# MAGIC-SCAN/adipose_tissue-unet

Hardware: AMD Instinct MI355X
Metric: 1024^2 tiles/sec (train) (higher is better)
Workload: dtype bf16; 1 GPU; unet_bn L5 base64 1024x1024x3 bf16 B=4/GPU (BASELINE configs[2]); preset=unet_bn, levels=5, tile=1024, batch_per_gpu=4, global_batch=4, parallelism=dp1

## Files before the change

### adipose_tissue-unet_amd/csrc/conv_fwd_halo.hip

```cpp
#include <type_traits>

#include "conv_common.h"

namespace {

__device__ __attribute__((aligned(256))) uint4 halo_zero_page[64];

constexpr int PH = 8, PW = 32;
constexpr int HH = PH + 2, HW = PW + 2;
constexpr int HROWS = HH * HW;
constexpr int ROWB = 128;

__device__ __forceinline__ int hswz(int r) { return r & 7; }

#define LDS_BAR()                                             \
  do {                                                        \
    asm volatile("s_waitcnt lgkmcnt(0)" ::: "memory");        \
    __builtin_amdgcn_s_barrier();                             \
    asm volatile("" ::: "memory");                            \
  } while (0)

#define HALO_BAR()                         \
  do {                                     \
    asm volatile("" ::: "memory");         \
    __builtin_amdgcn_s_barrier();          \
    asm volatile("" ::: "memory");         \
  } while (0)

template <int WN, int KS, int TPS, int NHB>
constexpr int halo_lds() {
  constexpr int NTH = 4 * WN * KS * 64;
  constexpr int GH = (HROWS * 8 + NTH - 1) / NTH;
  return NHB * (GH * NTH / 8) * ROWB + 3 * TPS * WN * 64 * ROWB;
}

template <int WN, int KS, int TPS, int NHB, bool BNR>
__global__ __launch_bounds__(4 * WN * KS * 64, (halo_lds<WN, KS, TPS, NHB>() <= 81920 ? 2 : 1))
void igemm_fwd_halo_kernel(FwdArgs a) {
  constexpr int NTH = 4 * WN * KS * 64;
  constexpr int BN = WN * 64;
  constexpr int SPC = (9 + TPS - 1) / TPS;
  constexpr int GH = (HROWS * 8 + NTH - 1) / NTH;
  constexpr int HROWS_PAD = GH * NTH / 8;
  constexpr int HBUF = HROWS_PAD * ROWB;
  constexpr int GB1 = BN * 8 / NTH;
  static_assert(GB1 * NTH == BN * 8, "weight slot must split evenly");
  constexpr int GB = GB1 * TPS;
  constexpr int WTAP = BN * ROWB;
  constexpr int WSLOT = TPS * WTAP;
  constexpr int OFF_W = NHB * HBUF;
  constexpr int LT = BN + 4;
  constexpr int EPI = PH * PW * LT * 4;
  constexpr int SMEM = (OFF_W + 3 * WSLOT > EPI) ? OFF_W + 3 * WSLOT : EPI;
  __shared__ __attribute__((aligned(1024))) unsigned char smem[SMEM];

  const int tid = threadIdx.x, lane = tid & 63;
  const int wave = __builtin_amdgcn_readfirstlane(tid >> 6);
  const int wm = wave % 4, wn = (wave / 4) % WN, kh = wave / (4 * WN);
  const int tx_n = a.Wo / PW, ty_n = a.Ho / PH;
  const int lin = xcd_remap(blockIdx.x, a.nblocks);
  const int tn = lin % a.ntile_n;
  int rest = lin / a.ntile_n;
  const int px = rest % tx_n; rest /= tx_n;
  const int py = rest % ty_n;
  const int img = rest / ty_n;
  const int y0 = py * PH, x0 = px * PW, n0 = tn * BN;
  const int Cin_s = a.CAs + a.CBs;
  const int nchunk = Cin_s / 64, nsteps = nchunk * SPC;
  const int Wrows = (a.Nout + 63) / 64 * 64;
  const bf16* srcA = reinterpret_cast<const bf16*>(a.srcA);
  const bf16* srcB = reinterpret_cast<const bf16*>(a.srcB);

  int hoff[GH], hcol[GH];
#pragma unroll
  for (int i = 0; i < GH; ++i) {
    const int idx = i * NTH + tid;
    const int hr = idx >> 3, pos = idx & 7;
    hcol[i] = 8 * (pos ^ hswz(hr));
    const int gy = y0 - 1 + hr / HW, gx = x0 - 1 + hr % HW;
    hoff[i] = (hr < HROWS && gy >= 0 && gy < a.Hs && gx >= 0 && gx < a.Ws) ? (img * a.Hs + gy) * a.Ws + gx : -1;
  }
  const bf16* wp[GB1];
#pragma unroll
  for (int i = 0; i < GB1; ++i) {
    const int idx = i * NTH + tid;
    const int q = idx >> 3, pos = idx & 7;
    wp[i] = (n0 + q < Wrows) ? reinterpret_cast<const bf16*>(a.W) + (size_t)(n0 + q) * a.Kpad + 8 * (pos ^ swz(q))
                             : nullptr;
  }

  auto issue_halo = [&](int c, int buf) {
    const int ci = c * 64;
    const bf16* base = ci < a.CAs ? srcA + ci : srcB + (ci - a.CAs);
    const int cs = ci < a.CAs ? a.CAs : a.CBs;
    unsigned char* dst = smem + buf * HBUF + wave * 8 * ROWB;
#pragma unroll
    for (int i = 0; i < GH; ++i) {
      const void* p = hoff[i] >= 0 ? (const void*)(base + (size_t)hoff[i] * cs + hcol[i]) : (const void*)halo_zero_page;
      __builtin_amdgcn_global_load_lds(p, (lds_void*)(dst + i * (NTH / 8) * ROWB), 16, 0, 0);
    }
  };
  auto issue_w = [&](int s) {
    const int c = s / SPC, j = s - SPC * c;
#pragma unroll
    for (int u = 0; u < TPS; ++u) {
      const int t = j * TPS + u;
      const int k = t * Cin_s + c * 64;
      unsigned char* dst = smem + OFF_W + (s % 3) * WSLOT + u * WTAP + wave * 8 * ROWB;
#pragma unroll
      for (int i = 0; i < GB1; ++i) {
        const void* p = (wp[i] && t < 9) ? (const void*)(wp[i] + k) : (const void*)halo_zero_page;
        __builtin_amdgcn_global_load_lds(p, (lds_void*)(dst + i * (NTH / 8) * ROWB), 16, 0, 0);
      }
    }
  };

  f32x4 acc[4][4];
#pragma unroll
  for (int i = 0; i < 4; ++i)
#pragma unroll
    for (int j = 0; j < 4; ++j) acc[i][j] = f32x4{0.f, 0.f, 0.f, 0.f};

  const int r16 = lane & 15, h4 = lane >> 4;
  issue_halo(0, 0);
  issue_w(0);
  if (nsteps > 1) {
    issue_w(1);
    asm volatile("s_waitcnt vmcnt(%0)" ::"n"(GB) : "memory");
  } else {
    asm volatile("s_waitcnt vmcnt(0)" ::: "memory");
  }
  HALO_BAR();

  for (int s = 0; s < nsteps; ++s) {
    const int c = s / SPC, j = s - SPC * c;
    const bool nh = NHB == 2 && j == 0 && c + 1 < nchunk;
    if (nh) issue_halo(c + 1, (c + 1) & 1);
    const bool nw = s + 2 < nsteps;
    if (nw) issue_w(s + 2);
    const unsigned char* H = smem + (NHB == 2 ? (c & 1) : 0) * HBUF;
#pragma unroll
    for (int u = 0; u < TPS; ++u) {
    const int t = j * TPS + u;
    if (t >= 9) break;
    const int dy = t / 3, dx = t - 3 * dy;
    const unsigned char* Wt = smem + OFF_W + (s % 3) * WSLOT + u * WTAP;
#pragma unroll
    for (int kq = 0; kq < 2 / KS; ++kq) {
      const int ck = 4 * (KS == 2 ? kh : kq) + h4;
      bf16x8 fb[4], fa[4];
#pragma unroll
      for (int nf = 0; nf < 4; ++nf) {
        const int q = wn * 64 + nf * 16 + r16;
        fb[nf] = *reinterpret_cast<const bf16x8*>(Wt + q * ROWB + ((ck ^ swz(q)) << 4));
      }
#pragma unroll
      for (int mf = 0; mf < 4; ++mf) {
        const int prow = 2 * wm + (mf >> 1), pcol = (mf & 1) * 16 + r16;
        const int hr = (prow + dy) * HW + pcol + dx;
        fa[mf] = *reinterpret_cast<const bf16x8*>(H + hr * ROWB + ((ck ^ hswz(hr)) << 4));
      }
#pragma unroll
      for (int mf = 0; mf < 4; ++mf)
#pragma unroll
        for (int nf = 0; nf < 4; ++nf)
          acc[mf][nf] = __builtin_amdgcn_mfma_f32_16x16x32_bf16(fa[mf], fb[nf], acc[mf][nf], 0, 0, 0);
    }
    }
    if (nw) {
      if (nh) asm volatile("s_waitcnt vmcnt(%0)" ::"n"(GB + GH) : "memory");
      else asm volatile("s_waitcnt vmcnt(%0)" ::"n"(GB) : "memory");
    } else {
      asm volatile("s_waitcnt vmcnt(0)" ::: "memory");
    }
    HALO_BAR();
  }

  float* tile = reinterpret_cast<float*>(smem);
  const int col = lane & 15, rq = (lane >> 4) * 4;
#pragma unroll
  for (int part = 0; part < KS; ++part) {
    if (kh == part) {
#pragma unroll
      for (int mf = 0; mf < 4; ++mf)
#pragma unroll
        for (int nf = 0; nf < 4; ++nf)
#pragma unroll
          for (int r = 0; r < 4; ++r) {
            const int p = (2 * wm + (mf >> 1)) * PW + (mf & 1) * 16 + rq + r;
            float* e = tile + p * LT + wn * 64 + nf * 16 + col;
            *e = part == 0 ? acc[mf][nf][r] : *e + acc[mf][nf][r];
          }
    }
    ADP_LDS_BARRIER();
  }
  float bs[8], bq[8];
#pragma unroll
  for (int j = 0; j < 8; ++j) { bs[j] = 0.f; bq[j] = 0.f; }
  for (int pr = 0; pr < PH; ++pr) {
    const int m0 = (img * a.Ho + y0 + pr) * a.Wo + x0;
    if constexpr (BNR) epi_rows_bnr<NTH, BN>(a, tile + pr * PW * LT, PW, m0, n0, tid, bs, bq);
    else epi_rows<NTH, BN>(a, tile + pr * PW * LT, PW, m0, n0, tid, bs, bq);
  }
  if (a.bn_sum || a.bnr_z) epi_bn_flush<NTH, BN>(a, tile, n0, tid, bs, bq);
}

#ifndef HALOP_VALU_PER_MFMA
#define HALOP_VALU_PER_MFMA 8
#endif
template <int I, int N, typename F>
__device__ __forceinline__ void halop_static_for(F&& f) {
  if constexpr (I < N) {
    f(std::integral_constant<int, I>{});
    halop_static_for<I + 1, N>(f);
  }
}
template <bool BNR, int NCH, int BN, bool PIPE, int EPI_, bool WIDE = false, bool DYN = false, bool SWP = false>
__global__ __launch_bounds__(512, 1) void igemm_fwd_halop_kernel(FwdArgs a) {
  constexpr bool BNL = EPI_ == 6;
  constexpr int EPI = BNL ? 1 : EPI_;
  static_assert(!BNL || (!BNR && !DYN && !SWP && NCH == 1), "BN-on-load: one-chunk static-list forward launches");
  static_assert(!BNR || EPI == 0, "the BN-backward reduction launch stores the plain product");
  static_assert(EPI < 4 || !PIPE, "mask / addend quads, the dropout hash and two accumulator sets: registers");
  constexpr int NTH = 512, NF = BN / 16;
  constexpr int HCH = NCH * HROWS * 8;
  constexpr int GH = (HCH + NTH - 1) / NTH;
  static_assert(!BNL || GH <= 6, "BN-on-load: at most six halo chunks per thread");
  constexpr int HBUF = HCH * 16;
  constexpr int GW = 9 * NCH * BN * 8 / NTH;
  constexpr int WTAP = NCH * BN * ROWB;
  constexpr int OFF_W = HBUF, OFF_C = OFF_W + 9 * WTAP;
  constexpr int OFF_S = OFF_C + 5 * BN * 4 + 16;
  constexpr int SMEM = OFF_S + (BNL ? 2 * NCH * 64 * 4 : 0);
  static_assert(GW * NTH == 9 * NCH * BN * 8, "weights must split evenly");
  static_assert(SMEM <= 160 * 1024, "LDS");
  typedef __bf16 bf16x4 __attribute__((ext_vector_type(4)));
  typedef unsigned int v2u32_h __attribute__((ext_vector_type(2)));
  typedef unsigned int v4u32_h __attribute__((ext_vector_type(4)));
  __shared__ __attribute__((aligned(1024))) unsigned char smem[SMEM];

  const int tid = threadIdx.x, lane = tid & 63;
  const int wave = __builtin_amdgcn_readfirstlane(tid >> 6);
  prio_static<ADP_PRIO_FWD>(wave);
  const int tx_n = a.Wo / PW, ty_n = a.Ho / PH;
  const int T = a.nblocks, G = gridDim.x;
  const int lin = xcd_remap(blockIdx.x, G);
  constexpr bool dyn = DYN;
  const bool full = dyn && a.claim_full;
  const int nt = dyn ? 0 : (lin < T ? (T - lin + G - 1) / G : 0);
  if (!dyn && nt == 0) return;
  const int Wrows = (a.Nout + 63) / 64 * 64;
  const int NT = a.ntile_n;
  const int nh = lin % NT, n0 = BN * nh;
  const bool second = a.out_mode == 2 && n0 >= a.split_c;
  bf16* obase = reinterpret_cast<bf16*>(second ? a.out2 : a.out);
  const int ostride = second ? a.out2_stride : a.out_stride;
  const int ocol0 = second ? n0 - a.split_c : n0;
  const int nlim = a.out_mode == 2 && !second ? a.split_c : a.Nout;
  const int Cin_s = a.CAs + a.CBs;

  int* ring = reinterpret_cast<int*>(smem + OFF_C + 5 * BN * 4);
  const int npatch = T / NT;
  const int CH = dyn ? a.claim_chunk : 1, nsup = (npatch + CH - 1) / CH;
  auto sup_id = [&](int sidx) -> int {
    const int v = full ? claim_ring_read(ring + (sidx & 3))
                       : sidx < 2 ? lin / NT + sidx * (G / NT) : 2 * (G / NT) + claim_ring_read(ring + (sidx & 3));
    return v < nsup ? v : -1;
  };
  auto tile_id = [&](int k) -> int {
    if (!dyn) return k < nt ? lin / NT + k * (G / NT) : -1;
    const int v = sup_id(k / CH);
    const int t = v * CH + k % CH;
    return v >= 0 && t < npatch ? t : -1;
  };
  if (full) {
    if (tid == 0) {
      const int r = claim_next2(a.claim + nh);
      ring[0] = r;
      ring[1] = r + 1;
    }
    __syncthreads();
  }
  if (dyn && tile_id(0) < 0) {
    if (tid == 0) claim_block_done(a.claim, NT, G);
    return;
  }
  auto tile_origin = [&](int t, int& img, int& y0, int& x0) {
    const int px = t % tx_n, r = t / tx_n;
    y0 = (r % ty_n) * PH;
    img = r / ty_n;
    x0 = px * PW;
  };
  auto halo_src = [&](int img, int y0, int x0, int i) -> const uint4* {
    const int idx = i * NTH + tid;
    const int cc = NCH == 1 ? 0 : (idx >= HROWS * 8 ? 1 : 0), hr = (idx - cc * HROWS * 8) >> 3;
    const int hy = hr / HW, hx = hr - hy * HW;
    const int gy = y0 + hy - 1, gx = x0 + hx - 1, us = a.up >> 1;
    const bool ok = (i < GH - 1 || idx < HCH) && (unsigned)gy < (unsigned)(a.Hs << us) && (unsigned)gx < (unsigned)(a.Ws << us);
    if (!ok) return nullptr;
    const bool inA = cc * 64 < a.CAs;
    const bf16* src = reinterpret_cast<const bf16*>(inA ? a.srcA : a.srcB);
    const int cs = inA ? a.CAs : a.CBs;
    return reinterpret_cast<const uint4*>(src + (size_t)((img * a.Hs + (gy >> us)) * a.Ws + (gx >> us)) * cs +
                                          (inA ? cc * 64 : cc * 64 - a.CAs) + 8 * ((tid & 7) ^ hswz(hr)));
  };

  const float* sS = reinterpret_cast<const float*>(smem + OFF_S);
  const bool act_w = BNL && n0 == 0 && a.act_out != nullptr && !(ADP_DBG(a) & 4096);
  const __amdgpu_buffer_rsrc_t rsA = __builtin_amdgcn_make_buffer_rsrc(
      a.act_out, 0, act_w ? a.Nimg * a.Hs * a.Ws * a.CAs * 2 : 0, 0x00020000);
  auto bnl = [&](uint4 v, int img, int y0, int x0, int i) -> uint4 {
    const int idx = i * NTH + tid;
    const int cc = NCH == 1 ? 0 : (idx >= HROWS * 8 ? 1 : 0), hr = (idx - cc * HROWS * 8) >> 3;
    const int hy = hr / HW, hx = hr - hy * HW;
    const int gy = y0 + hy - 1, gx = x0 + hx - 1;
    const bool inimg = (unsigned)gy < (unsigned)a.Hs && (unsigned)gx < (unsigned)a.Ws;
    const int c0 = cc * 64 + 8 * ((tid & 7) ^ hswz(hr));
    Grp<bf16> g;
    g.v = v;
    bf16* e = reinterpret_cast<bf16*>(&g.v);
#pragma unroll
    for (int hv = 0; hv < 2; ++hv) {
      const float4 q = *reinterpret_cast<const float4*>(sS + c0 + 4 * hv);
      const float4 r = *reinterpret_cast<const float4*>(sS + NCH * 64 + c0 + 4 * hv);
      e[4 * hv + 0] = (bf16)fmaxf(fmaf((float)e[4 * hv + 0], q.x, r.x), 0.f);
      e[4 * hv + 1] = (bf16)fmaxf(fmaf((float)e[4 * hv + 1], q.y, r.y), 0.f);
      e[4 * hv + 2] = (bf16)fmaxf(fmaf((float)e[4 * hv + 2], q.z, r.z), 0.f);
      e[4 * hv + 3] = (bf16)fmaxf(fmaf((float)e[4 * hv + 3], q.w, r.w), 0.f);
    }
    const bool wr = inimg && hy >= 1 && hy <= PH && hx >= 1 && hx <= PW;
    const unsigned off = wr ? (unsigned)((((img * a.Hs + gy) * a.Ws + gx) * a.CAs + c0) * 2) : 0x80000000u;
    if (act_w) __builtin_amdgcn_raw_buffer_store_b128(__builtin_bit_cast(v4u32_h, g.v), rsA, off, 0, 0);
    return inimg ? g.v : v;
  };

#pragma unroll
  for (int i = 0; i < GW; ++i) {
    const int idx = i * NTH + tid;
    const int tc = idx / (BN * 8), rem = idx - tc * BN * 8;
    const int t = tc / NCH, cc = tc - t * NCH;
    const int q = rem >> 3, pos = rem & 7;
    const void* p = n0 + q < Wrows
                        ? (const void*)(reinterpret_cast<const bf16*>(a.W) + (size_t)(n0 + q) * a.Kpad + t * Cin_s + cc * 64 +
                                        8 * (pos ^ swz(q)))
                        : (const void*)halo_zero_page;
    __builtin_amdgcn_global_load_lds(p, (lds_void*)(smem + OFF_W + (size_t)(i * NTH + wave * 64) * 16), 16, 0, 0);
  }
  int img0, y00, x00;
  tile_origin(tile_id(0), img0, y00, x00);
#pragma unroll
  for (int i = 0; i < GH; ++i) {
    if (i * NTH + tid < HCH) {
      const uint4* p = halo_src(img0, y00, x00, i);
      __builtin_amdgcn_global_load_lds(p ? (const void*)p : (const void*)halo_zero_page,
                                       (lds_void*)(smem + (size_t)(i * NTH + wave * 64) * 16), 16, 0, 0);
    }
  }
  float* cst = reinterpret_cast<float*>(smem + OFF_C);
  if (tid < BN) {
    const int c = n0 + tid;
    const bool v = c < a.Nout;
    cst[tid] = (!BNR && a.bias && v) ? a.bias[c] : 0.f;
    cst[BN + tid] = (BNR && v) ? a.bnr_sc[c] : 0.f;
    cst[2 * BN + tid] = (BNR && v) ? a.bnr_sh[c] : 0.f;
    cst[3 * BN + tid] = (BNR && v) ? -a.bnr_mean[c] * a.bnr_invstd[c] : 0.f;
    cst[4 * BN + tid] = (BNR && v) ? a.bnr_invstd[c] : 0.f;
  }
  if constexpr (BNL) {
    float* sw = reinterpret_cast<float*>(smem + OFF_S);
    if (tid < NCH * 64) {
      sw[tid] = a.scA[tid];
      sw[NCH * 64 + tid] = a.shA[tid];
    }
  }
  asm volatile("s_waitcnt vmcnt(0)" ::: "memory");
  __syncthreads();
  if constexpr (BNL) {
#pragma unroll
    for (int i = 0; i < GH; ++i)
      if (i * NTH + tid < HCH) {
        uint4* q = reinterpret_cast<uint4*>(smem + (size_t)(i * NTH + tid) * 16);
        *q = bnl(*q, img0, y00, x00, i);
      }
    __syncthreads();
  }

  const int r16 = lane & 15, h4 = lane >> 4;
  constexpr bool stats = BNR || EPI == 1 || EPI == 3;
  float s1[NF][4], s2[NF][4];
#pragma unroll
  for (int nf = 0; nf < NF; ++nf)
#pragma unroll
    for (int i = 0; i < 4; ++i) { s1[nf][i] = 0.f; s2[nf][i] = 0.f; }

  const __amdgpu_buffer_rsrc_t rsO =
      __builtin_amdgcn_make_buffer_rsrc((void*)obase, 0, a.M * ostride * 2, 0x00020000);
  const __amdgpu_buffer_rsrc_t rsZ = __builtin_amdgcn_make_buffer_rsrc(
      (void*)(BNR ? a.bnr_z : a.out), 0, BNR ? a.M * a.bnr_zs * 2 : 0, 0x00020000);
  const void* mptr = second ? a.mask2 : a.mask;
  const int mstr = second ? a.mask2_stride : a.mask_stride;
  const float mscale = second ? a.mask2_scale : a.mask_scale;
  const bool has_mask = EPI == 4 && mptr != nullptr, has_add = EPI == 4 && !second && a.addend != nullptr;
  const __amdgpu_buffer_rsrc_t rsM =
      __builtin_amdgcn_make_buffer_rsrc((void*)mptr, 0, has_mask ? a.M * mstr * 2 : 0, 0x00020000);
  const __amdgpu_buffer_rsrc_t rsD =
      __builtin_amdgcn_make_buffer_rsrc((void*)a.addend, 0, has_add ? a.M * a.addend_stride * 2 : 0, 0x00020000);
  auto load_q = [&](__amdgpu_buffer_rsrc_t rs, int str, int col0, int mrow_, uint2 (&zr)[2][NF]) {
#pragma unroll
    for (int mf = 0; mf < 2; ++mf)
#pragma unroll
      for (int nf = 0; nf < NF; ++nf) {
        const int c0 = nf * 16 + 4 * h4;
        const unsigned off = n0 + c0 < nlim ? (unsigned)(((mrow_ + mf * 16 + r16) * str + col0 + c0) * 2) : 0x80000000u;
        zr[mf][nf] = __builtin_bit_cast(uint2, __builtin_amdgcn_raw_buffer_load_b64(rs, off, 0, 0));
      }
  };
  auto load_z = [&](int mrow_, uint2 (&zr)[2][NF]) {
    if (ADP_DBG(a) & 8192) {
#pragma unroll
      for (int mf = 0; mf < 2; ++mf)
#pragma unroll
        for (int nf = 0; nf < NF; ++nf) zr[mf][nf] = uint2{0u, 0u};
      return;
    }
    load_q(rsZ, a.bnr_zs, n0, mrow_, zr);
  };
  auto epi_vals = [&](int mf, int nf, const f32x4& av, uint2 zv, int mrow_, uint2 dv = uint2{0u, 0u}) -> bf16x4 {
    const int c0 = nf * 16 + 4 * h4;
    const float4 cb = *reinterpret_cast<const float4*>(cst + c0);
    const int m = mrow_ + mf * 16 + r16;
    float v[4] = {av[0] + cb.x, av[1] + cb.y, av[2] + cb.z, av[3] + cb.w};
    if constexpr (EPI == 4) {
      const bf16x4 dd = __builtin_bit_cast(bf16x4, dv), mm = __builtin_bit_cast(bf16x4, zv);
#pragma unroll
      for (int i = 0; i < 4; ++i) {
        if (has_add) v[i] += (float)dd[i];
        if (has_mask) v[i] = (float)mm[i] > 0.f ? v[i] * mscale : 0.f;
      }
    }
    if constexpr (EPI == 5) {
      const float ks = 1.f / (1.f - a.drop_rate);
#pragma unroll
      for (int i = 0; i < 4; ++i) {
        const float u = adp_uniform(a.drop_seed, (uint64_t)m * (uint64_t)a.Nout + (n0 + c0 + i));
        v[i] = u >= a.drop_rate ? fmaxf(v[i], 0.f) * ks : 0.f;
      }
    }
    bf16x4 o;
#pragma unroll
    for (int i = 0; i < 4; ++i) {
      if constexpr (EPI == 2 || EPI == 3) v[i] = fmaxf(v[i], 0.f);
      o[i] = (bf16)v[i];
    }
    if constexpr (BNR) {
      if (ADP_DBG(a) & 16384) return o;
      const float4 sc = *reinterpret_cast<const float4*>(cst + BN + c0);
      const float4 sh = *reinterpret_cast<const float4*>(cst + 2 * BN + c0);
      const float4 nm = *reinterpret_cast<const float4*>(cst + 3 * BN + c0);
      const float4 is = *reinterpret_cast<const float4*>(cst + 4 * BN + c0);
      const float scv[4] = {sc.x, sc.y, sc.z, sc.w}, shv[4] = {sh.x, sh.y, sh.z, sh.w};
      const float nmv[4] = {nm.x, nm.y, nm.z, nm.w}, isv[4] = {is.x, is.y, is.z, is.w};
      bf16x4 zz = __builtin_bit_cast(bf16x4, zv);
#pragma unroll
      for (int i = 0; i < 4; ++i) {
        const float g = (float)o[i], zf = (float)zz[i];
        const float db = fmaf(zf, scv[i], shv[i]) > 0.f ? g : 0.f;
        s1[nf][i] += db;
        s2[nf][i] = fmaf(db, fmaf(zf, isv[i], nmv[i]), s2[nf][i]);
      }
    } else if constexpr (EPI == 1 || EPI == 3) {
#pragma unroll
      for (int i = 0; i < 4; ++i) {
        s1[nf][i] += v[i];
        s2[nf][i] = fmaf(v[i], v[i], s2[nf][i]);
      }
    }
    return o;
  };
  auto epi_unit = [&](int mf, int nf, const f32x4& av, uint2 zv, int mrow_, uint2 dv = uint2{0u, 0u}) {
    const bf16x4 o = epi_vals(mf, nf, av, zv, mrow_, dv);
    const int c0 = nf * 16 + 4 * h4, m = mrow_ + mf * 16 + r16;
    const unsigned off = n0 + c0 < nlim ? (unsigned)((m * ostride + ocol0 + c0) * 2) : 0x80000000u;
    __builtin_amdgcn_raw_buffer_store_b64(__builtin_bit_cast(v2u32_h, o), rsO, off, 0, 0);
  };
  auto epi_join = [&](int mf, int nf, v2u32_h o0, v2u32_h o1, int mrow_) {
    const auto e0 = __builtin_amdgcn_permlane16_swap(o0.x, o1.x, false, false);
    const auto e1 = __builtin_amdgcn_permlane16_swap(o0.y, o1.y, false, false);
    const v4u32_h st = {e0[0], e1[0], e0[1], e1[1]};
    const int cw = 16 * (nf + (h4 & 1)) + 8 * (h4 >> 1), m = mrow_ + mf * 16 + r16;
    const unsigned off = n0 + cw < nlim ? (unsigned)((m * ostride + ocol0 + cw) * 2) : 0x80000000u;
    __builtin_amdgcn_raw_buffer_store_b128(st, rsO, off, 0, 0);
  };
  auto epi_pair = [&](int mf, int nf, const f32x4& av0, const f32x4& av1, uint2 zv0, uint2 zv1, int mrow_,
                      uint2 dv0 = uint2{0u, 0u}, uint2 dv1 = uint2{0u, 0u}) {
    const v2u32_h o0 = __builtin_bit_cast(v2u32_h, epi_vals(mf, nf, av0, zv0, mrow_, dv0));
    const v2u32_h o1 = __builtin_bit_cast(v2u32_h, epi_vals(mf, nf + 1, av1, zv1, mrow_, dv1));
    epi_join(mf, nf, o0, o1, mrow_);
  };
  v2u32_h pend = {0u, 0u};
  auto epi_all = [&](const f32x4 (&av)[2][NF], const uint2 (&zv)[2][NF], int mrow_, const uint2 (&dv)[EPI == 4 ? 2 : 1][NF]) {
    if constexpr (WIDE) {
#pragma unroll
      for (int nf = 0; nf < NF; nf += 2)
#pragma unroll
        for (int mf = 0; mf < 2; ++mf)
          epi_pair(mf, nf, av[mf][nf], av[mf][nf + 1], zv[mf][nf], zv[mf][nf + 1], mrow_, dv[EPI == 4 ? mf : 0][nf],
                   dv[EPI == 4 ? mf : 0][nf + 1]);
    } else {
#pragma unroll
      for (int nf = 0; nf < NF; ++nf)
#pragma unroll
        for (int mf = 0; mf < 2; ++mf) epi_unit(mf, nf, av[mf][nf], zv[mf][nf], mrow_, dv[EPI == 4 ? mf : 0][nf]);
    }
  };

  f32x4 acc[2][NF], accp[2][NF];
  uint2 zreg[2][NF], dreg[EPI == 4 ? 2 : 1][NF];
  int mrowp = 0;
  auto load_halo = [&](int t, uint4 (&hr)[GH]) {
    int img1, y01, x01;
    tile_origin(t, img1, y01, x01);
    const bool nohalo = (ADP_DBG(a) & 1024) != 0;
#pragma unroll
    for (int i = 0; i < GH; ++i) {
      const uint4* p = nohalo ? nullptr : halo_src(img1, y01, x01, i);
      hr[i] = p ? *p : make_uint4(0, 0, 0, 0);
    }
  };
  auto run_tile = [&](int k, int tk, auto with_prev, uint4 (&hreg)[GH]) -> int {
    constexpr bool EPI_PREV = decltype(with_prev)::value;
    if constexpr (!DYN) tk = tile_id(k);
    const int tn = tile_id(k + 1);
    const bool more = tn >= 0;
    const bool claim_now = dyn && k % CH == 0 && more && sup_id(k / CH + 1) >= 0;
    int claimed = 0;
    if (claim_now && tid == 0) claimed = __hip_atomic_fetch_add(a.claim + nh, 1, __ATOMIC_RELAXED, __HIP_MEMORY_SCOPE_AGENT);
    int img, y0, x0;
    tile_origin(tk, img, y0, x0);
    const int mrow = (img * a.Ho + y0 + wave) * a.Wo + x0;
    if constexpr (BNR) load_z(EPI_PREV ? mrowp : mrow, zreg);
    if constexpr (EPI == 4) {
      if (has_mask) load_q(rsM, mstr, ocol0, mrow, zreg);
      if (has_add) load_q(rsD, a.addend_stride, ocol0, mrow, dreg);
    }
    if (more) load_halo(DYN ? tn : tile_id(k + 1), hreg);
    int img1 = 0, y01 = 0, x01 = 0;
    if constexpr (BNL) {
      if (more) tile_origin(tn, img1, y01, x01);
    }
#pragma unroll
    for (int i = 0; i < 2; ++i)
#pragma unroll
      for (int j = 0; j < NF; ++j) acc[i][j] = f32x4{0.f, 0.f, 0.f, 0.f};
    if constexpr (SWP) {
      constexpr int NS = 18 * NCH;
      bf16x8 FB[2][NF], FA[2][2];
      auto ldf = [&](auto sc, bf16x8 (&fb)[NF], bf16x8 (&fa)[2]) {
        constexpr int st = decltype(sc)::value, t = st / (2 * NCH), cc = (st >> 1) % NCH, kq = st & 1;
        constexpr int dy = t / 3, dx = t - 3 * dy;
        const unsigned char* Wt = smem + OFF_W + t * WTAP + cc * BN * ROWB;
        const unsigned char* Hc = smem + cc * HROWS * ROWB;
        const int ck = 4 * kq + h4;
#pragma unroll
        for (int nf = 0; nf < NF; ++nf) {
          const int q = nf * 16 + r16;
          fb[nf] = *reinterpret_cast<const bf16x8*>(Wt + q * ROWB + ((ck ^ swz(q)) << 4));
        }
#pragma unroll
        for (int mf = 0; mf < 2; ++mf) {
          const int hr = (wave + dy) * HW + mf * 16 + r16 + dx;
          fa[mf] = *reinterpret_cast<const bf16x8*>(Hc + hr * ROWB + ((ck ^ hswz(hr)) << 4));
        }
      };
      ldf(std::integral_constant<int, 0>{}, FB[0], FA[0]);
      halop_static_for<0, NS>([&](auto sc) {
        constexpr int st = decltype(sc)::value, t = st / (2 * NCH), cc = (st >> 1) % NCH, kq = st & 1;
        if constexpr (st + 1 < NS) ldf(std::integral_constant<int, st + 1>{}, FB[(st + 1) & 1], FA[(st + 1) & 1]);
        __builtin_amdgcn_sched_barrier(0);
        const bf16x8(&fb)[NF] = FB[st & 1];
        const bf16x8(&fa)[2] = FA[st & 1];
        constexpr bool with_unit = EPI_PREV && cc == 0 && kq == 0 && t >= 1 && t - 1 < 2 * NF;
        if constexpr (with_unit) {
          constexpr int u = t - 1;
          if constexpr (WIDE) {
            constexpr int p = u >> 1, mf = p & 1, nf = 2 * (p >> 1);
            if constexpr ((u & 1) == 0) {
              pend = __builtin_bit_cast(v2u32_h, epi_vals(mf, nf, accp[mf][nf], zreg[mf][nf], mrowp));
            } else {
              epi_join(mf, nf, pend, __builtin_bit_cast(v2u32_h, epi_vals(mf, nf + 1, accp[mf][nf + 1],
                                                                          zreg[mf][nf + 1], mrowp)), mrowp);
            }
          } else {
            epi_unit(u & 1, u >> 1, accp[u & 1][u >> 1], zreg[u & 1][u >> 1], mrowp);
          }
        }
        if constexpr (!with_unit) prio_hi<ADP_PRIO_FWD>();
#pragma unroll
        for (int mf = 0; mf < 2; ++mf)
#pragma unroll
          for (int nf = 0; nf < NF; ++nf)
            acc[mf][nf] = __builtin_amdgcn_mfma_f32_16x16x32_bf16(fb[nf], fa[mf], acc[mf][nf], 0, 0, 0);
        if constexpr (!with_unit) prio_lo<ADP_PRIO_FWD>();
        if constexpr (with_unit) {
#pragma unroll
          for (int i = 0; i < 2 * NF; ++i) {
            __builtin_amdgcn_sched_group_barrier(0x008, 1, 0);
            __builtin_amdgcn_sched_group_barrier(0x002, HALOP_VALU_PER_MFMA, 0);
          }
        }
      });
    }
#pragma unroll
    for (int t = 0; t < (SWP ? 0 : 9); ++t) {
      const int dy = t / 3, dx = t - 3 * dy;
#pragma unroll
      for (int cc = 0; cc < NCH; ++cc) {
        const unsigned char* Wt = smem + OFF_W + t * WTAP + cc * BN * ROWB;
        const unsigned char* Hc = smem + cc * HROWS * ROWB;
#pragma unroll
        for (int kq = 0; kq < 2; ++kq) {
          const int ck = 4 * kq + h4;
          bf16x8 fb[NF], fa[2];
#pragma unroll
          for (int nf = 0; nf < NF; ++nf) {
            const int q = nf * 16 + r16;
            fb[nf] = *reinterpret_cast<const bf16x8*>(Wt + q * ROWB + ((ck ^ swz(q)) << 4));
          }
#pragma unroll
          for (int mf = 0; mf < 2; ++mf) {
            const int hr = (wave + dy) * HW + mf * 16 + r16 + dx;
            fa[mf] = *reinterpret_cast<const bf16x8*>(Hc + hr * ROWB + ((ck ^ hswz(hr)) << 4));
          }
          constexpr bool unit_here = EPI_PREV;
          const bool with_unit = unit_here && cc == 0 && kq == 0 && t >= 1 && t - 1 < 2 * NF;
          if (with_unit) {
            const int u = t - 1;
            if constexpr (WIDE) {
              const int p = u >> 1, mf = p & 1, nf = 2 * (p >> 1);
              if ((u & 1) == 0) {
                pend = __builtin_bit_cast(v2u32_h, epi_vals(mf, nf, accp[mf][nf], zreg[mf][nf], mrowp));
              } else {
                epi_join(mf, nf, pend, __builtin_bit_cast(v2u32_h, epi_vals(mf, nf + 1, accp[mf][nf + 1],
                                                                            zreg[mf][nf + 1], mrowp)), mrowp);
              }
            } else {
              const int mf = u & 1, nf = u >> 1;
              epi_unit(mf, nf, accp[mf][nf], zreg[mf][nf], mrowp);
            }
          }
          const bool with_apply = BNL && kq == 1 && t >= 3 && t - 3 < GH;
          if constexpr (BNL) {
            if (with_apply && more) hreg[t - 3] = bnl(hreg[t - 3], img1, y01, x01, t - 3);
          }
          if (!with_unit && !with_apply) prio_hi<ADP_PRIO_FWD>();
#pragma unroll
          for (int mf = 0; mf < 2; ++mf)
#pragma unroll
            for (int nf = 0; nf < NF; ++nf)
              acc[mf][nf] = __builtin_amdgcn_mfma_f32_16x16x32_bf16(fb[nf], fa[mf], acc[mf][nf], 0, 0, 0);
          if (!with_unit && !with_apply) prio_lo<ADP_PRIO_FWD>();
          if (with_unit || with_apply) {
#pragma unroll
            for (int i = 0; i < 2 * NF; ++i) {
              __builtin_amdgcn_sched_group_barrier(0x008, 1, 0);
              __builtin_amdgcn_sched_group_barrier(0x002, HALOP_VALU_PER_MFMA, 0);
            }
          }
        }
      }
    }
    if constexpr (PIPE) {
#pragma unroll
      for (int i = 0; i < 2; ++i)
#pragma unroll
        for (int j = 0; j < NF; ++j) accp[i][j] = acc[i][j];
      mrowp = mrow;
    } else {
      epi_all(acc, zreg, mrow, dreg);
    }
    if (more) {
      LDS_BAR();
#pragma unroll
      for (int i = 0; i < GH; ++i)
        if (i * NTH + tid < HCH) *reinterpret_cast<uint4*>(smem + (size_t)(i * NTH + tid) * 16) = hreg[i];
      if (claim_now && tid == 0) ring[(k / CH + 2) & 3] = claimed;
      LDS_BAR();
    }
    return DYN ? tn : tile_id(k + 1);
  };
  uint4 hA[GH];
  int tnext = run_tile(0, tile_id(0), std::false_type{}, hA);
  for (int k = 1; tnext >= 0; ++k) tnext = run_tile(k, tnext, std::integral_constant<bool, PIPE>{}, hA);
  if constexpr (PIPE) {
    if constexpr (BNR) load_z(mrowp, zreg);
    epi_all(accp, zreg, mrowp, dreg);
  }
  if (dyn && tid == 0) claim_block_done(a.claim, NT, G);
  if (!stats || (ADP_DBG(a) & 2)) return;
  double* d0 = a.stat + (size_t)((blockIdx.x * 8 + wave) & (adp::STAT_REPL - 1)) * 2 * adp::STAT_CMAX;
#pragma unroll
  for (int nf = 0; nf < NF; ++nf)
#pragma unroll
    for (int i = 0; i < 4; ++i) {
      const float x = row16_sum(s1[nf][i]), y = row16_sum(s2[nf][i]);
      const int c = n0 + nf * 16 + 4 * h4 + i;
      if (r16 == 0 && c < a.Nout) {
        atomicAdd(d0 + c, (double)x);
        atomicAdd(d0 + adp::STAT_CMAX + c, (double)y);
      }
    }
}

#undef HALO_BAR
#undef LDS_BAR

template <int WN, int KS, int TPS, int NHB>
void launch_halo(FwdArgs& a, hipStream_t s) {
  constexpr int BN = WN * 64;
  a.ntile_n = (a.Nout + BN - 1) / BN;
  a.nblocks = a.Nimg * (a.Ho / PH) * (a.Wo / PW) * a.ntile_n;
  adp::set_kernel("igemm_fwd_halo_kernel<%d, %d, %d, %d, %s>", WN, KS, TPS, NHB, a.bnr_z ? "true" : "false");
  const dim3 g(a.nblocks), b(4 * WN * KS * 64);
  if (a.bnr_z) hipLaunchKernelGGL((igemm_fwd_halo_kernel<WN, KS, TPS, NHB, true>), g, b, 0, s, a);
  else hipLaunchKernelGGL((igemm_fwd_halo_kernel<WN, KS, TPS, NHB, false>), g, b, 0, s, a);
}

}

namespace adp {
int launch_fwd_halo(FwdArgs& a, hipStream_t s) {
  const int mode = option("fwd_halo", 1);
  if (mode == 0) return 0;
  const int Cin_s = a.CAs + a.CBs;
  const bool bnl = a.scA != nullptr;
  if (bnl && !(a.act_out && a.CBs == 0 && a.up == 1 && a.CAs == 64 && a.bn_sum && !a.bnr_z &&
               !a.relu && !a.bias && option("halop_bnl", 1)))
    return 0;
  if (a.scB || a.kh != 3 || a.kw != 3 || a.dil != 1 || a.pad != 1 || a.stride != 1 || (a.up != 1 && a.up != 2) ||
      a.Ho != a.Hs * a.up || a.Wo != a.Ws * a.up || a.Ho % PH != 0 || a.Wo % PW != 0 || a.CAs % 64 != 0 || a.CBs % 64 != 0 ||
      a.K != 9 * Cin_s || a.Kpad != a.K || a.Nout > 128)
    return 0;
  if (a.bnr_z && (a.out_mode != 0 || a.bias || a.relu || a.drop_rate > 0.f || a.accum || a.bn_sum)) return 0;
  const bool one_chunk = Cin_s == 64;
  const bool plain = !a.addend && !a.mask && !a.mask2 && !a.accum && a.drop_rate == 0.f && a.out_stride % 8 == 0;
  const bool dropepi = a.drop_rate > 0.f && a.relu && !a.addend && !a.mask && !a.mask2 && !a.accum && !a.bn_sum &&
                       !a.bnr_z && a.out_mode == 0 && a.out_stride % 8 == 0 && option("halop_dropout", 1);
  const bool maskepi = (a.addend || a.mask || a.mask2) && !a.accum && a.drop_rate == 0.f && !a.bnr_z && !a.bn_sum && !a.relu && !a.bias &&
                       a.out_stride % 8 == 0 && (!a.mask || a.mask_stride % 4 == 0) &&
                       (!a.mask2 || a.mask2_stride % 4 == 0) && (!a.addend || a.addend_stride % 4 == 0) &&
                       (size_t)a.M * std::max(std::max(a.mask ? a.mask_stride : 0, a.mask2 ? a.mask2_stride : 0),
                                              a.addend ? a.addend_stride : 0) * 2 < ((size_t)1 << 31) &&
                       option("halop_mask", 1);
  int bn = 0;
  if (one_chunk && (a.Nout <= 64 || a.Nout == 128)) bn = 64;
  else if (Cin_s == 128 && (a.Nout == 64 || a.Nout == 128) && option("halo_persist2", 1)) bn = 32;
  const int nt_n = bn ? (a.Nout + bn - 1) / bn : 1;
  const bool split_ok = a.out_mode == 2 && bn && a.split_c > 0 && a.split_c % bn == 0 && a.split_c < a.Nout &&
                        (!a.mask2 || maskepi) && a.out2_stride % 8 == 0 && (a.Nout - a.split_c) % bn == 0;
  const size_t lim = (size_t)1 << 31;
  const bool fits = (size_t)a.M * a.out_stride * 2 < lim && (!a.out2 || (size_t)a.M * a.out2_stride * 2 < lim) &&
                    (!a.bnr_z || (size_t)a.M * a.bnr_zs * 2 < lim);
  if (bn && (plain || maskepi || dropepi) && fits && (a.out_mode == 0 || split_ok) && option("halo_persist", 1) &&
      (a.up == 1 || !a.bnr_z)) {
    const int tiles = a.Nimg * (a.Ho / PH) * (a.Wo / PW) * nt_n;
    a.ntile_n = nt_n;
    a.nblocks = tiles;
    int grid = std::max(1, std::min(tiles, option("halo_persist_grid", 256)));
    grid -= grid % nt_n;
    if (grid == 0) grid = nt_n;
    const bool bnr = a.bnr_z != nullptr;
    const int pm = option("halop_pipe", 1);
    const int swm = option("halop_swp", 2);
    const bool swp_req = !bnr && !dropepi && (swm == 1 || (swm == 2 && !one_chunk));
    const bool pipe = !swp_req && !bnr && !maskepi && !dropepi && (pm == 2 || (pm == 1 && one_chunk));
    const int epi = bnr ? 0 : dropepi ? 5 : maskepi ? 4 : (a.bn_sum ? 1 : 0) + (a.relu ? 2 : 0);
    const int wm = option("halop_wide", 3);
    const bool wide = !bnr && (wm == 2 || (wm == 1 && !pipe) || (wm == 3 && !(pipe && (epi == 1 || epi == 3)))) &&
                      a.Nout % 8 == 0 && (a.out_mode != 2 || a.split_c % 8 == 0);
    a.claim = option("halop_claim", option("dp_claim", 0)) && nt_n + 1 <= CLAIM_INTS && !(bnr && one_chunk) && !(pipe && (epi == 1 || epi == 3))
                  ? claim_slot() : nullptr;
    a.claim_chunk = std::max(1, option("halop_claim_chunk", 4));
    a.claim_full = 0;
    if (a.claim) {
      const int nsup = (tiles / nt_n + a.claim_chunk - 1) / a.claim_chunk;
      grid = std::max(nt_n, std::min(grid, nsup * nt_n));
      a.claim_full = option("claim_full", 0) && nsup >= 4 * (grid / nt_n);
    }
    if (bnl) a.claim = nullptr;
    const bool dyn = a.claim != nullptr;
    const bool swp = !dyn && swp_req;
    if (bnl) {
      if (one_chunk && a.Nout <= 64 && pipe && !wide && !swp && epi == 1) {
        adp::set_kernel("igemm_fwd_halop_kernel<false, 1, 64, true, 6, false, false, false>");
        hipLaunchKernelGGL((igemm_fwd_halop_kernel<false, 1, 64, true, 6, false, false, false>), dim3(grid), dim3(512), 0,
                           s, a);
        return 1;
      }
      return 0;
    }
    adp::set_kernel("igemm_fwd_halop_kernel<%s, %d, %d, %s, %d, %s, %s, %s>", bnr ? "true" : "false", one_chunk ? 1 : 2, bn,
                    pipe ? "true" : "false", epi, wide ? "true" : "false", dyn ? "true" : "false", swp ? "true" : "false");
#define HALOP_LAUNCH_WD(NCH_, BN_, W_, D_, P_)                                                                   \
  do {                                                                                                      \
    if (bnr) hipLaunchKernelGGL((igemm_fwd_halop_kernel<true, NCH_, BN_, false, 0, false, D_, P_>), dim3(grid), dim3(512), 0, s, a); \
    else if (epi == 4) hipLaunchKernelGGL((igemm_fwd_halop_kernel<false, NCH_, BN_, false, 4, W_, D_, P_>), dim3(grid), dim3(512), 0, s, a); \
    else if (epi == 5) hipLaunchKernelGGL((igemm_fwd_halop_kernel<false, NCH_, BN_, false, 5, W_, D_, P_>), dim3(grid), dim3(512), 0, s, a); \
    else if (pipe) {                                                                                        \
      if (epi == 1) hipLaunchKernelGGL((igemm_fwd_halop_kernel<false, NCH_, BN_, true, 1, W_, D_, P_>), dim3(grid), dim3(512), 0, s, a); \
      else if (epi == 2) hipLaunchKernelGGL((igemm_fwd_halop_kernel<false, NCH_, BN_, true, 2, W_, D_, P_>), dim3(grid), dim3(512), 0, s, a); \
      else if (epi == 3) hipLaunchKernelGGL((igemm_fwd_halop_kernel<false, NCH_, BN_, true, 3, W_, D_, P_>), dim3(grid), dim3(512), 0, s, a); \
      else hipLaunchKernelGGL((igemm_fwd_halop_kernel<false, NCH_, BN_, true, 0, W_, D_, P_>), dim3(grid), dim3(512), 0, s, a); \
    } else {                                                                                                \
      if (epi == 1) hipLaunchKernelGGL((igemm_fwd_halop_kernel<false, NCH_, BN_, false, 1, W_, D_, P_>), dim3(grid), dim3(512), 0, s, a); \
      else if (epi == 2) hipLaunchKernelGGL((igemm_fwd_halop_kernel<false, NCH_, BN_, false, 2, W_, D_, P_>), dim3(grid), dim3(512), 0, s, a); \
      else if (epi == 3) hipLaunchKernelGGL((igemm_fwd_halop_kernel<false, NCH_, BN_, false, 3, W_, D_, P_>), dim3(grid), dim3(512), 0, s, a); \
      else hipLaunchKernelGGL((igemm_fwd_halop_kernel<false, NCH_, BN_, false, 0, W_, D_, P_>), dim3(grid), dim3(512), 0, s, a); \
    }                                                                                                       \
  } while (0)
#define HALOP_LAUNCH_SWP(NCH_, BN_, W_)                                                                         \
  do {                                                                                                      \
    if (epi == 4) hipLaunchKernelGGL((igemm_fwd_halop_kernel<false, NCH_, BN_, false, 4, W_, false, true>), dim3(grid), dim3(512), 0, s, a); \
    else if (epi == 1) hipLaunchKernelGGL((igemm_fwd_halop_kernel<false, NCH_, BN_, false, 1, W_, false, true>), dim3(grid), dim3(512), 0, s, a); \
    else if (epi == 2) hipLaunchKernelGGL((igemm_fwd_halop_kernel<false, NCH_, BN_, false, 2, W_, false, true>), dim3(grid), dim3(512), 0, s, a); \
    else if (epi == 3) hipLaunchKernelGGL((igemm_fwd_halop_kernel<false, NCH_, BN_, false, 3, W_, false, true>), dim3(grid), dim3(512), 0, s, a); \
    else hipLaunchKernelGGL((igemm_fwd_halop_kernel<false, NCH_, BN_, false, 0, W_, false, true>), dim3(grid), dim3(512), 0, s, a); \
  } while (0)
#define HALOP_LAUNCH_W(NCH_, BN_, W_)                          \
  do {                                                         \
    if (dyn) HALOP_LAUNCH_WD(NCH_, BN_, W_, true, false);      \
    else if (swp) HALOP_LAUNCH_SWP(NCH_, BN_, W_);              \
    else HALOP_LAUNCH_WD(NCH_, BN_, W_, false, false);         \
  } while (0)
#define HALOP_LAUNCH(NCH_, BN_)                  \
  do {                                           \
    if (wide) HALOP_LAUNCH_W(NCH_, BN_, true);   \
    else HALOP_LAUNCH_W(NCH_, BN_, false);       \
  } while (0)
    if (one_chunk) HALOP_LAUNCH(1, 64);
    else HALOP_LAUNCH(2, 32);
#undef HALOP_LAUNCH_W
#undef HALOP_LAUNCH_WD
#undef HALOP_LAUNCH_SWP
#undef HALOP_LAUNCH
    return 1;
  }
  if (bnl) return 0;
  if (a.Nout == 128 && Cin_s > 128 && !a.bnr_z && plain && a.out_mode != 1 && option("halo_defer_tap64p", 1))
    return 0;
  if (a.up != 1) return 0;
  if (a.Nout <= 64) {
    if (one_chunk && mode != 2) launch_halo<1, 2, 1, 1>(a, s);
    else launch_halo<1, 2, 2, 2>(a, s);
  } else {
    if (one_chunk && mode != 2) launch_halo<2, 1, 1, 1>(a, s);
    else launch_halo<2, 1, 1, 2>(a, s);
  }
  return 1;
}
}
```

Before: 181.8 tiles/s.

## Double-buffer halo tiles in LDS via direct global-to-LDS loads

Adds a two-slot LDS halo buffer for one-chunk, BN=64, static-list forward conv launches. The next tile's halo is loaded with global_load_lds straight into the alternate slot, replacing the register staging and the LDS write-back that sat behind a barrier. The aim is to overlap halo fetch with the current tile's MFMA work and to save VGPRs. Per-channel bias is also cached in registers. In exchange it doubles halo LDS usage and relies on vmcnt accounting around the epilogue stores, and it is enabled by default only for the stats and BN-reduction epilogues.

After: 182.4 tiles/s, median of 6. No clear change (+0.3%).

```diff
diff --git a/adipose_tissue-unet_amd/csrc/conv_fwd_halo.hip b/adipose_tissue-unet_amd/csrc/conv_fwd_halo.hip
--- a/adipose_tissue-unet_amd/csrc/conv_fwd_halo.hip
+++ b/adipose_tissue-unet_amd/csrc/conv_fwd_halo.hip
@@ -208,6 +208,9 @@
 #ifndef HALOP_VALU_PER_MFMA
 #define HALOP_VALU_PER_MFMA 8
 #endif
+#define HALOP_DMA2_AUTO_PLAIN false
+#define HALOP_DMA2_AUTO_STATS true
+#define HALOP_DMA2_AUTO_BNR true
 template <int I, int N, typename F>
 __device__ __forceinline__ void halop_static_for(F&& f) {
   if constexpr (I < N) {
@@ -215,9 +218,11 @@
     halop_static_for<I + 1, N>(f);
   }
 }
-template <bool BNR, int NCH, int BN, bool PIPE, int EPI_, bool WIDE = false, bool DYN = false, bool SWP = false>
+template <bool BNR, int NCH, int BN, bool PIPE, int EPI_, bool WIDE = false, bool DYN = false, bool SWP = false, int... RING>
 __global__ __launch_bounds__(512, 1) void igemm_fwd_halop_kernel(FwdArgs a) {
+  constexpr bool DMA2 = sizeof...(RING) != 0;
   constexpr bool BNL = EPI_ == 6;
+  static_assert(!DMA2 || (NCH == 1 && BN == 64 && !DYN && !SWP && !BNL), "two halo slots: one-chunk static-list forms");
   constexpr int EPI = BNL ? 1 : EPI_;
   static_assert(!BNL || (!BNR && !DYN && !SWP && NCH == 1), "BN-on-load: one-chunk static-list forward launches");
   static_assert(!BNR || EPI == 0, "the BN-backward reduction launch stores the plain product");
@@ -229,7 +234,7 @@
   constexpr int HBUF = HCH * 16;
   constexpr int GW = 9 * NCH * BN * 8 / NTH;
   constexpr int WTAP = NCH * BN * ROWB;
-  constexpr int OFF_W = HBUF, OFF_C = OFF_W + 9 * WTAP;
+  constexpr int OFF_W = (DMA2 ? 2 : 1) * HBUF, OFF_C = OFF_W + 9 * WTAP;
   constexpr int OFF_S = OFF_C + 5 * BN * 4 + 16;
   constexpr int SMEM = OFF_S + (BNL ? 2 * NCH * 64 * 4 : 0);
   static_assert(GW * NTH == 9 * NCH * BN * 8, "weights must split evenly");
@@ -387,6 +392,12 @@
 
   const int r16 = lane & 15, h4 = lane >> 4;
   constexpr bool stats = BNR || EPI == 1 || EPI == 3;
+  constexpr bool CBREG = DMA2 && !BNR;
+  float4 cbr[CBREG ? NF : 1];
+  if constexpr (CBREG) {
+#pragma unroll
+    for (int nf = 0; nf < NF; ++nf) cbr[nf] = *reinterpret_cast<const float4*>(cst + nf * 16 + 4 * h4);
+  }
   float s1[NF][4], s2[NF][4];
 #pragma unroll
   for (int nf = 0; nf < NF; ++nf)
@@ -427,7 +438,7 @@
   };
   auto epi_vals = [&](int mf, int nf, const f32x4& av, uint2 zv, int mrow_, uint2 dv = uint2{0u, 0u}) -> bf16x4 {
     const int c0 = nf * 16 + 4 * h4;
-    const float4 cb = *reinterpret_cast<const float4*>(cst + c0);
+    const float4 cb = CBREG ? cbr[CBREG ? nf : 0] : *reinterpret_cast<const float4*>(cst + c0);
     const int m = mrow_ + mf * 16 + r16;
     float v[4] = {av[0] + cb.x, av[1] + cb.y, av[2] + cb.z, av[3] + cb.w};
     if constexpr (EPI == 4) {
@@ -526,6 +537,22 @@
       const uint4* p = nohalo ? nullptr : halo_src(img1, y01, x01, i);
       hr[i] = p ? *p : make_uint4(0, 0, 0, 0);
     }
+  };
+  auto issue_halo = [&](int t, int slot) {
+    int img1, y01, x01;
+    tile_origin(t, img1, y01, x01);
+    if (!(ADP_DBG(a) & 1024)) {
+#pragma unroll
+      for (int i = 0; i < GH; ++i) {
+        if (i * NTH + tid < HCH) {
+          const uint4* p = halo_src(img1, y01, x01, i);
+          __builtin_amdgcn_global_load_lds(p ? (const void*)p : (const void*)halo_zero_page,
+                                           (lds_void*)(smem + (size_t)slot * HBUF + (size_t)(i * NTH + wave * 64) * 16), 16,
+                                           0, 0);
+        }
+      }
+    }
+    asm volatile("" ::: "memory");
   };
   auto run_tile = [&](int k, int tk, auto with_prev, uint4 (&hreg)[GH]) -> int {
     constexpr bool EPI_PREV = decltype(with_prev)::value;
@@ -543,7 +570,13 @@
       if (has_mask) load_q(rsM, mstr, ocol0, mrow, zreg);
       if (has_add) load_q(rsD, a.addend_stride, ocol0, mrow, dreg);
     }
-    if (more) load_halo(DYN ? tn : tile_id(k + 1), hreg);
+    if constexpr (DMA2) {
+      asm volatile("" ::: "memory");
+      if (more) issue_halo(tn, (k + 1) & 1);
+    } else {
+      if (more) load_halo(DYN ? tn : tile_id(k + 1), hreg);
+    }
+    const unsigned char* Hs = smem + (DMA2 ? (k & 1) * HBUF : 0);
     int img1 = 0, y01 = 0, x01 = 0;
     if constexpr (BNL) {
       if (more) tile_origin(tn, img1, y01, x01);
@@ -559,7 +592,7 @@
         constexpr int st = decltype(sc)::value, t = st / (2 * NCH), cc = (st >> 1) % NCH, kq = st & 1;
         constexpr int dy = t / 3, dx = t - 3 * dy;
         const unsigned char* Wt = smem + OFF_W + t * WTAP + cc * BN * ROWB;
-        const unsigned char* Hc = smem + cc * HROWS * ROWB;
+        const unsigned char* Hc = Hs + cc * HROWS * ROWB;
         const int ck = 4 * kq + h4;
 #pragma unroll
         for (int nf = 0; nf < NF; ++nf) {
@@ -616,7 +649,7 @@
 #pragma unroll
       for (int cc = 0; cc < NCH; ++cc) {
         const unsigned char* Wt = smem + OFF_W + t * WTAP + cc * BN * ROWB;
-        const unsigned char* Hc = smem + cc * HROWS * ROWB;
+        const unsigned char* Hc = Hs + cc * HROWS * ROWB;
 #pragma unroll
         for (int kq = 0; kq < 2; ++kq) {
           const int ck = 4 * kq + h4;
@@ -678,7 +711,14 @@
     } else {
       epi_all(acc, zreg, mrow, dreg);
     }
-    if (more) {
+    if constexpr (DMA2) {
+      if (more) {
+        constexpr int NSTORE = WIDE ? NF : 2 * NF;
+        if constexpr (PIPE && !EPI_PREV) asm volatile("s_waitcnt vmcnt(0)" ::: "memory");
+        else asm volatile("s_waitcnt vmcnt(%0)" ::"n"(NSTORE) : "memory");
+        LDS_BAR();
+      }
+    } else if (more) {
       LDS_BAR();
 #pragma unroll
       for (int i = 0; i < GH; ++i)
@@ -798,6 +838,31 @@
       }
       return 0;
     }
+    const int dm = option("halop_dma2", 2);
+    const bool dma2_has = one_chunk && !dyn && !swp && (bnr || (pipe && epi < 4));
+    const bool dma2_auto = bnr ? HALOP_DMA2_AUTO_BNR : (epi == 1 || epi == 3) ? HALOP_DMA2_AUTO_STATS : HALOP_DMA2_AUTO_PLAIN;
+    if (dma2_has && (dm == 1 || (dm == 2 && dma2_auto))) {
+      const bool p2 = !bnr, w2 = !bnr && wide;
+      adp::set_kernel("igemm_fwd_halop_kernel<%s, %d, %d, %s, %d, %s, %s, %s, 1>", bnr ? "true" : "false", 1, 64,
+                      p2 ? "true" : "false", epi, w2 ? "true" : "false", "false", "false");
+#define HALOP_DMA2_LAUNCH(B_, P_, E_, W_) \
+  hipLaunchKernelGGL((igemm_fwd_halop_kernel<B_, 1, 64, P_, E_, W_, false, false, 1>), dim3(grid), dim3(512), 0, s, a)
+      if (bnr) {
+        HALOP_DMA2_LAUNCH(true, false, 0, false);
+      } else if (wide) {
+        if (epi == 1) HALOP_DMA2_LAUNCH(false, true, 1, true);
+        else if (epi == 2) HALOP_DMA2_LAUNCH(false, true, 2, true);
+        else if (epi == 3) HALOP_DMA2_LAUNCH(false, true, 3, true);
+        else HALOP_DMA2_LAUNCH(false, true, 0, true);
+      } else {
+        if (epi == 1) HALOP_DMA2_LAUNCH(false, true, 1, false);
+        else if (epi == 2) HALOP_DMA2_LAUNCH(false, true, 2, false);
+        else if (epi == 3) HALOP_DMA2_LAUNCH(false, true, 3, false);
+        else HALOP_DMA2_LAUNCH(false, true, 0, false);
+      }
+#undef HALOP_DMA2_LAUNCH
+      return 1;
+    }
     adp::set_kernel("igemm_fwd_halop_kernel<%s, %d, %d, %s, %d, %s, %s, %s>", bnr ? "true" : "false", one_chunk ? 1 : 2, bn,
                     pipe ? "true" : "false", epi, wide ? "true" : "false", dyn ? "true" : "false", swp ? "true" : "false");
 #define HALOP_LAUNCH_WD(NCH_, BN_, W_, D_, P_)                                                                   \
```
